# Prayforhanluo/HiCHap_master

Measured on NVIDIA B200. Metric: matrix_stage_time_to_ice_convergence, lower is better.
Workload: dtype int32 counts (ICE streams them as u8 + overflow list, s32 tensor-core plane sums) / f64 weights

## Files before the change

### hichap_master_b200/csrc/hc_ice.cu

```cuda
#include <cooperative_groups.h>
#include <vector>
#include <algorithm>
#include <math.h>
#include <stdlib.h>
#include "hc_common.cuh"
#include "hc_select.cuh"

namespace {

__device__ __forceinline__ double band_weight(int j, int r, int kd) {
    const int d = j - r;
    if (d == 0) return kd == 0 ? 2.0 : 0.0;
    return (d < kd && d > -kd) ? 0.0 : 1.0;
}

__global__ void __launch_bounds__(256)
ice_dense_marginals_kernel(const int32_t* __restrict__ mats, const int64_t* __restrict__ mat_off,
                           const int32_t* __restrict__ mat_n, const int32_t* __restrict__ mat_ld,
                           const int64_t* __restrict__ bin_off, int nprob, int kd,
                           double* __restrict__ nnz_marg, double* __restrict__ marg) {
    const int64_t g = ((int64_t)blockIdx.x * blockDim.x + threadIdx.x) >> 5;
    const int lane = threadIdx.x & 31;
    if (g >= bin_off[nprob]) return;
    int p = 0;
// ... 216 lines not shown
    }
    if (!mad_last_cta(st, &flag_s)) return;
    if (threadIdx.x == 0) {
        const long long k = mad_median_rank(count);
        const long long le_all = *reinterpret_cast<volatile long long*>(&st->le);
        const unsigned long long nxt_all = *reinterpret_cast<volatile unsigned long long*>(&st->nxt);
        const double lo = key_f64(klo);
        double hi = lo;
        if (k + 1 < count && le_all < k + 2) hi = key_f64(nxt_all);
        st->result[STAGE] = (count & 1) ? lo : __dmul_rn(__dadd_rn(lo, hi), 0.5);
    }
}

__global__ void __launch_bounds__(MAD_THREADS)
mad_apply_kernel(const double* __restrict__ marg, long long n, double mad_max, const MadState* __restrict__ st,
                 double* __restrict__ bias) {
    const double cutoff = exp(__dadd_rn(st->result[0], -__dmul_rn(mad_max, st->result[1])));
    for (long long i = (long long)blockIdx.x * blockDim.x + threadIdx.x; i < n; i += (long long)gridDim.x * blockDim.x)
        if (marg[i] < cutoff) bias[i] = 0.0;
}

struct IceDenseArgs {
    const int32_t* mats; const int64_t* mat_off; const int32_t* mat_n; const int32_t* mat_ld;
    const int64_t* pad_off;
    const int32_t* item_prob; const int32_t* item_row0; const int32_t* item_nrows;
    const unsigned int* nitems; unsigned int* queue;
    int32_t* iter;
    double* bias;
    double* marg;
    hc_ice_result* results; int32_t* done; int32_t* n_done;
    double tol; int kd; int max_iters; int nprob;
    unsigned int queue_start;
    const uint8_t* q8; const int64_t* q_off;
    uint8_t* digits; int32_t* dig_exp;
    const int4* desc; int kseg;
    double* part; int nseg_max; long long npad;
    const int64_t* bin_off;
    const int64_t* ovf_ptr; const int32_t* ovf_col; const int32_t* ovf_val;
    int packed;
};

template <int RG>
__device__ __forceinline__ void consume_chunk(const int4 (&a)[RG], const double* __restrict__ b, int j, int jc,
                                              int rg, int kd, int kspan, double (&acc)[RG]) {
    const double2 b01 = *reinterpret_cast<const double2*>(b + j);
    const double2 b23 = *reinterpret_cast<const double2*>(b + j + 2);
    const bool band = jc <= rg + RG - 1 + kspan && jc + 127 >= rg - kspan;
#pragma unroll
    for (int q = 0; q < RG; ++q) {
        double x0 = (double)a[q].x, x1 = (double)a[q].y, x2 = (double)a[q].z, x3 = (double)a[q].w;
        if (band) {
            const int r = rg + q;
            x0 *= band_weight(j, r, kd); x1 *= band_weight(j + 1, r, kd);
            x2 *= band_weight(j + 2, r, kd); x3 *= band_weight(j + 3, r, kd);
        }
        acc[q] = fma(x0, b01.x, acc[q]); acc[q] = fma(x1, b01.y, acc[q]);
        acc[q] = fma(x2, b23.x, acc[q]); acc[q] = fma(x3, b23.y, acc[q]);
    }
}

template <int RG, int U, int MINB>
__global__ void __launch_bounds__(256, MINB)
ice_dense_stream_kernel(IceDenseArgs A) {
    const int lane = threadIdx.x & 31;
    const int kd = A.kd, kspan = kd > 0 ? kd - 1 : 0;
    const unsigned nitems = *A.nitems;
// ... 33 lines not shown
                        for (int q = 0; q < RG; ++q) a[u][q] = ld_stream_v4(base + roff[q] + (c0 + u) * 128);
#pragma unroll
                    for (int u = 0; u < U; ++u)
                        consume_chunk<RG>(a[u], b, (c0 + u) * 128 + 4 * lane, (c0 + u) * 128, rg, kd, kspan, acc);
                }
                for (; c0 < nchunk; ++c0) {
                    int4 a[RG];
#pragma unroll
                    for (int q = 0; q < RG; ++q) a[q] = ld_stream_v4(base + roff[q] + c0 * 128);
                    consume_chunk<RG>(a, b, c0 * 128 + 4 * lane, c0 * 128, rg, kd, kspan, acc);
                }
#pragma unroll
                for (int q = 0; q < RG; ++q) {
                    const double sacc = warp_sum(acc[q]);
                    if (lane == 0 && q < nr) mout[rg + q] = b[rg + q] * sacc;
                }
            }
        }
        item = __shfl_sync(0xffffffffu, next, 0);
    }
}

__device__ __forceinline__ long long weighted_count(int v, int j, int r, int kd) {
    const int d = j - r;
    if (d == 0) return kd == 0 ? 2ll * v : 0ll;
    return (d < kd && d > -kd) ? 0ll : (long long)v;
}

__global__ void __launch_bounds__(256)
ice_pack_tiles_kernel(const int32_t* __restrict__ mats, const int64_t* __restrict__ mat_off,
                      const int32_t* __restrict__ mat_n, const int32_t* __restrict__ mat_ld,
                      const int64_t* __restrict__ q_off, const int64_t* __restrict__ strip_off,
                      const int64_t* __restrict__ bin_off, int nprob, int kd, uint8_t* __restrict__ q8,
                      unsigned long long* __restrict__ ovf_cnt, int32_t* __restrict__ ovf_lo, int32_t* __restrict__ ovf_hi) {
    const int64_t gs = ((int64_t)blockIdx.x * blockDim.x + threadIdx.x) >> 5;
    const int lane = threadIdx.x & 31;
    if (gs >= strip_off[nprob]) return;
    int p = 0;
    while (p + 1 < nprob && strip_off[p + 1] <= gs) ++p;
    const int sidx = (int)(gs - strip_off[p]), n = mat_n[p], ld = mat_ld[p], KT = ld >> 5;
    const int32_t* M = mats + mat_off[p];
    uint8_t* out = q8 + q_off[p] + (int64_t)sidx * KT * 512 + 16 * lane;
    const int g = lane >> 2, c = 4 * (lane & 3);
    const int ra = sidx * 16 + g, rb = ra + 8;
    const int64_t grow = bin_off[p] + sidx * 16;
    for (int t = 8 * blockIdx.y; t < min(KT, 8 * (int)blockIdx.y + 8); ++t) {
        uint32_t w[4];
#pragma unroll
        for (int h = 0; h < 4; ++h) {
            const int r = (h & 1) ? rb : ra, j0 = t * 32 + ((h & 2) ? 16 : 0) + c;
            uint32_t word = 0;
            if (r < n) {
                const int4 a = ld_stream_v4(M + (int64_t)r * ld + j0);
                const int x[4] = {a.x, a.y, a.z, a.w};
#pragma unroll
                for (int e = 0; e < 4; ++e) {
                    const long long wc = (j0 + e < n) ? weighted_count(x[e], j0 + e, r, kd) : 0ll;
                    if (wc > 255) {
                        const int64_t gr = grow + (r - sidx * 16);
                        atomicAdd(ovf_cnt + gr, 1ull);
                        atomicMin(ovf_lo + gr, j0 + e);
                        atomicMax(ovf_hi + gr, j0 + e);
                    }
                    word |= (uint32_t)(wc > 255 ? 255 : (wc < 0 ? 0 : wc)) << (8 * e);
                }
            }
            w[h] = word;
        }
        *reinterpret_cast<uint4*>(out + (int64_t)t * 512) = make_uint4(w[0], w[1], w[2], w[3]);
    }
}

__device__ __forceinline__ void ice_store_digits(const double (&bv)[4], int j4, double pow2, uint32_t* __restrict__ dw) {
    unsigned long long F[4];
#pragma unroll
    for (int e = 0; e < 4; ++e) F[e] = bv[e] > 0.0 ? __double2ull_rn(bv[e] * pow2) : 0ull;
    const int t = j4 >> 5, cc = j4 & 31, sub = (cc & 15) >> 2, reg = cc >> 4;
#pragma unroll
    for (int pl = 0; pl < 8; ++pl) {
        const int sh = 8 * (7 - pl);
        const uint32_t word = (uint32_t)((F[0] >> sh) & 255ull) | ((uint32_t)((F[1] >> sh) & 255ull) << 8) |
                              ((uint32_t)((F[2] >> sh) & 255ull) << 16) | ((uint32_t)((F[3] >> sh) & 255ull) << 24);
        dw[t * 64 + (pl * 4 + sub) * 2 + reg] = word;
    }
}

__device__ __forceinline__ double block_max(double v, double* red) {
#pragma unroll
    for (int o = 16; o > 0; o >>= 1) v = fmax(v, __shfl_xor_sync(0xffffffffu, v, o));
    __syncthreads();
    if ((threadIdx.x & 31) == 0) red[threadIdx.x >> 5] = v;
    __syncthreads();
    double t = 0.0;
    for (int w = 0; w < (int)(blockDim.x >> 5); ++w) t = fmax(t, red[w]);
    return t;
}

__device__ __forceinline__ int digits_exponent(double mx, double* pow2) {
    const int E = (mx > 1.0e-300 && mx < 1.0e300) ? (int)((__double_as_longlong(mx) >> 52) & 0x7ff) - 1023 + 1 : 0;
    *pow2 = __longlong_as_double((long long)(1023 + 64 - E) << 52);
    return E;
}
// ... 79 lines not shown
                    int32_t* __restrict__ ovf_col, int32_t* __restrict__ ovf_val) {
    const int64_t g = ((int64_t)blockIdx.x * blockDim.x + threadIdx.x) >> 5;
    const int lane = threadIdx.x & 31;
    if (g >= bin_off[nprob]) return;
    int64_t out = ovf_ptr[g];
    if (ovf_ptr[g + 1] == out) return;
    int p = 0;
    while (p + 1 < nprob && bin_off[p + 1] <= g) ++p;
    const int r = (int)(g - bin_off[p]);
    const int32_t* row = mats + mat_off[p] + (int64_t)r * mat_ld[p];
    const int hi = ovf_hi[g];
    for (int j0 = ovf_lo[g]; j0 <= hi; j0 += 32) {
        const int j = j0 + lane;
        const long long w = j <= hi ? weighted_count(row[j], j, r, kd) : 0ll;
        const unsigned m = __ballot_sync(0xffffffffu, w > 255);
        if (w > 255) {
            const int64_t at = out + __popc(m & ((1u << lane) - 1u));
            ovf_col[at] = j;
            ovf_val[at] = (int32_t)(w - 255);
        }
        out += __popc(m);
    }
}

__device__ __forceinline__ void mma_u8(int (&c)[4], const int4& a, const uint2& b) {
    asm volatile("mma.sync.aligned.m16n8k32.row.col.s32.u8.u8.s32 {%0,%1,%2,%3}, {%4,%5,%6,%7}, {%8,%9}, {%0,%1,%2,%3};"
                 : "+r"(c[0]), "+r"(c[1]), "+r"(c[2]), "+r"(c[3])
                 : "r"(a.x), "r"(a.y), "r"(a.z), "r"(a.w), "r"(b.x), "r"(b.y));
}

template <int RS, int U, int MINB>
__global__ void __launch_bounds__(256, MINB)
ice_q8_mma_kernel(IceDenseArgs A) {
    const int lane = threadIdx.x & 31;
    const int g = lane >> 2, t4 = lane & 3;
    const double w_even = __longlong_as_double((long long)(1023 + 8 * (7 - 2 * t4)) << 52);
    const double w_odd = __longlong_as_double((long long)(1023 + 8 * (6 - 2 * t4)) << 52);
    const unsigned nitems = *A.nitems;
    unsigned cur = (blockIdx.x * 256u + threadIdx.x) >> 5;
    unsigned nxt = 0;
    if (lane == 0) {
        nxt = atomicAdd(A.queue, 1u);
        if (cur == 0) atomicAdd(A.iter, 1);
    }
    int4 d0 = make_int4(0, 0, 0, 0), d1 = d0, d2 = d0, d3 = d0;
    if (cur < nitems) {
        const int4* dp = A.desc + 4 * (int64_t)A.item_prob[cur];
        d0 = __ldg(dp); d1 = __ldg(dp + 1); d2 = __ldg(dp + 2); d3 = __ldg(dp + 3);
    }
    nxt = __shfl_sync(0xffffffffu, nxt, 0);
    while (cur < nitems) {
        unsigned drawn = 0;
        if (lane == 0) drawn = atomicAdd(A.queue, 1u);
        int4 e0 = make_int4(0, 0, 0, 0), e1 = e0, e2 = e0, e3 = e0;
        if (nxt < nitems) {
            const int4* dp = A.desc + 4 * (int64_t)A.item_prob[nxt];
            e0 = __ldg(dp); e1 = __ldg(dp + 1); e2 = __ldg(dp + 2); e3 = __ldg(dp + 3);
        }
        const int p = d2.x;
        if (!A.done[p]) {
            const int64_t tile_off = ((int64_t)(uint32_t)d0.x) | ((int64_t)d0.y << 32);
            const int64_t part_base = ((int64_t)(uint32_t)d0.z) | ((int64_t)d0.w << 32);
            const int64_t dig_off = ((int64_t)(uint32_t)d1.x) | ((int64_t)d1.y << 32);
            const int64_t grow = ((int64_t)(uint32_t)d1.z) | ((int64_t)d1.w << 32);
            const int nrows = d2.w, nk = d3.x, seg = d3.y, KT = d3.z;
            const uint8_t* qp = A.q8 + tile_off + 16 * lane;
            const uint8_t* dig = A.digits + dig_off + 8 * lane;
            const double* __restrict__ b = A.bias + d2.y;
            const double scale = __longlong_as_double((long long)(1023 + A.dig_exp[p] - 64) << 52);
            double* pout = A.part + part_base;
            const int ns = min(RS, (nrows + 15) >> 4);
            const uint8_t* sp[RS];
#pragma unroll
            for (int s = 0; s < RS; ++s) sp[s] = qp + (int64_t)min(s, ns - 1) * KT * 512;
            int c[RS][4];
#pragma unroll
            for (int s = 0; s < RS; ++s) { c[s][0] = 0; c[s][1] = 0; c[s][2] = 0; c[s][3] = 0; }
            for (int t = 0; t < nk; t += U) {
                int4 a[U][RS];
                uint2 bf[U];
#pragma unroll
                for (int u = 0; u < U; ++u) {
                    const int tt = min(t + u, nk - 1);
#pragma unroll
                    for (int s = 0; s < RS; ++s)
                        a[u][s] = ld_stream_v4(reinterpret_cast<const int32_t*>(sp[s] + (int64_t)tt * 512));
                    bf[u] = t + u < nk ? *reinterpret_cast<const uint2*>(dig + (int64_t)tt * 256) : make_uint2(0u, 0u);
                }
#pragma unroll
                for (int u = 0; u < U; ++u)
#pragma unroll
                    for (int s = 0; s < RS; ++s) mma_u8(c[s], a[u][s], bf[u]);
            }
#pragma unroll
            for (int s = 0; s < RS; ++s) {
                if (s < ns) {
                    const int ra = 16 * s + g, rb = ra + 8;
                    double va = ((double)c[s][0] * w_even + (double)c[s][1] * w_odd) * scale;
                    double vb = ((double)c[s][2] * w_even + (double)c[s][3] * w_odd) * scale;
                    if (seg == 0) {
                        if (ra < nrows) {
                            const int64_t x0 = A.ovf_ptr[grow + ra], x1 = A.ovf_ptr[grow + ra + 1];
                            for (int64_t e = x0 + t4; e < x1; e += 4) va = fma((double)A.ovf_val[e], b[A.ovf_col[e]], va);
                        }
                        if (rb < nrows) {
                            const int64_t x0 = A.ovf_ptr[grow + rb], x1 = A.ovf_ptr[grow + rb + 1];
                            for (int64_t e = x0 + t4; e < x1; e += 4) vb = fma((double)A.ovf_val[e], b[A.ovf_col[e]], vb);
                        }
                    }
                    va += __shfl_xor_sync(0xffffffffu, va, 1); va += __shfl_xor_sync(0xffffffffu, va, 2);
                    vb += __shfl_xor_sync(0xffffffffu, vb, 1); vb += __shfl_xor_sync(0xffffffffu, vb, 2);
                    if (t4 == 0) {
                        if (ra < nrows) pout[ra] = va;
                        if (rb < nrows) pout[rb] = vb;
                    }
                }
            }
        }
        cur = nxt; d0 = e0; d1 = e1; d2 = e2; d3 = e3;
        nxt = __shfl_sync(0xffffffffu, drawn, 0);
    }
}

__global__ void __launch_bounds__(1024)
ice_dense_update_kernel(IceDenseArgs A) {
    __shared__ double red[32];
    __shared__ long long redll[32];
    const int p = blockIdx.x;
    const int k = *A.iter;
    if (p == 0 && threadIdx.x == 0) *A.queue = A.queue_start;
    if (A.done[p] || k > A.max_iters) return;
    const int n = A.mat_n[p];
    if (n == 0) return;
    const int64_t lo = A.pad_off[p];
    double* m_in = A.marg + lo;
    double* bw = A.bias + lo;
    const double nan = __longlong_as_double(0x7ff8000000000000ll);
    if (A.packed && n <= 8 * (int)blockDim.x) {
        const int nseg = ((A.mat_ld[p] >> 5) + A.kseg - 1) / A.kseg;
        const int ld = A.mat_ld[p];
        const double* part = A.part + lo;
        double m[8], bb[8];
        double s = 0.0;
        long long c = 0;
        const int ja = 4 * threadIdx.x, jb = 4 * (int)blockDim.x + 4 * threadIdx.x;
        const bool ina = ja < ld, inb = jb < ld;
#pragma unroll
        for (int i = 0; i < 8; ++i) m[i] = 0.0;
#pragma unroll
// ... 239 lines not shown
    int p = 0;
    while (p + 1 < nprob && bin_off[p + 1] <= g) ++p;
    padded[pad_off[p] + (g - bin_off[p])] = bias[g];
}

__global__ void __launch_bounds__(256)
ice_finalize_kernel(const int64_t* __restrict__ bin_off, const int64_t* __restrict__ pad_off, int nprob,
                    const hc_ice_result* __restrict__ results, int rescale, const double* __restrict__ padded,
                    double* __restrict__ bias) {
    const int64_t g = (int64_t)blockIdx.x * blockDim.x + threadIdx.x;
    if (g >= bin_off[nprob]) return;
    int p = 0;
    while (p + 1 < nprob && bin_off[p + 1] <= g) ++p;
    const hc_ice_result r = results[p];
    const double nan = __longlong_as_double(0x7ff8000000000000ll);
    double b = padded[pad_off[p] + (g - bin_off[p])];
    if (isnan(r.scale)) b = nan;
    else {
        if (b == 0.0) b = nan;
        if (rescale) b = b / sqrt(r.scale);
    }
    bias[g] = b;
}

struct Scratch {
    cudaStream_t s;
    std::vector<void*> ptrs;
    explicit Scratch(cudaStream_t st) : s(st) {}
    cudaError_t alloc(void** p, size_t bytes) {
        const cudaError_t e = cudaMallocAsync(p, bytes, s);
        if (e == cudaSuccess) ptrs.push_back(*p);
        return e;
    }
    ~Scratch() { for (void* p : ptrs) cudaFreeAsync(p, s); }
};
struct EventPair {
    cudaEvent_t a = nullptr, b = nullptr;
    void create() { cudaEventCreate(&a); cudaEventCreate(&b); }
    ~EventPair() { if (a) cudaEventDestroy(a); if (b) cudaEventDestroy(b); }
};

typedef void (*StreamKernel)(IceDenseArgs);
struct StreamVariant { StreamKernel fn; int rg, u, minb; };
const StreamVariant kVariants[] = {
    {ice_dense_stream_kernel<4, 2, 4>, 4, 2, 4},
    {ice_dense_stream_kernel<4, 2, 3>, 4, 2, 3},
    {ice_dense_stream_kernel<2, 2, 4>, 2, 2, 4},
    {ice_dense_stream_kernel<2, 4, 3>, 2, 4, 3},
    {ice_dense_stream_kernel<4, 4, 2>, 4, 4, 2},
    {ice_dense_stream_kernel<1, 4, 4>, 1, 4, 4},
};

const StreamVariant kQ8Variants[] = {
    {ice_q8_mma_kernel<2, 4, 4>, 32, 4, 4},
    {ice_q8_mma_kernel<1, 4, 4>, 16, 4, 4},
    {ice_q8_mma_kernel<1, 8, 3>, 16, 8, 3},
    {ice_q8_mma_kernel<2, 4, 3>, 32, 4, 3},
    {ice_q8_mma_kernel<1, 8, 4>, 16, 8, 4},
    {ice_q8_mma_kernel<2, 8, 2>, 32, 8, 2},
    {ice_q8_mma_kernel<1, 16, 2>, 16, 16, 2},
    {ice_q8_mma_kernel<1, 12, 3>, 16, 12, 3},
};

}

extern "C" int hc_ice_dense_marginals(const int32_t* mats, const int64_t* mat_off, const int32_t* mat_n,
                                      const int32_t* mat_ld, const int64_t* bin_off, int32_t nprob,
                                      int32_t ignore_diags, double* nnz_marg, double* marg, void* stream) {
    HC_REQUIRE(nprob > 0 && ignore_diags >= 0, "nprob>0, ignore_diags>=0");
    int64_t total = 0;
    HC_CUDA(hc_read_small(&total, bin_off + nprob, sizeof(int64_t), (cudaStream_t)stream));
    if (total == 0) return HC_OK;
    const int64_t blocks = (total * 32 + 255) / 256;
    ice_dense_marginals_kernel<<<(unsigned)blocks, 256, 0, (cudaStream_t)stream>>>(
        mats, mat_off, mat_n, mat_ld, bin_off, nprob, ignore_diags, nnz_marg, marg);
    HC_LAUNCH_CHECK();
    return HC_OK;
}

extern "C" int hc_ice_filter_bins(const double* nnz_marg, double* marg, int64_t nbins, const int64_t* chrom_off,
                                  int32_t nchrom, const hc_ice_params* P, double* bias, double* work, void* stream) {
    HC_REQUIRE(nbins >= 0 && nchrom > 0 && P != nullptr, "nbins>=0, nchrom>0, params");
    if (nbins == 0) return HC_OK;
    const int do_mad = P->mad_max > 0.0;
    ice_filter_chrom_kernel<<<nchrom, 1024, 0, (cudaStream_t)stream>>>(nnz_marg, marg, chrom_off, P->min_nnz,
                                                                      P->min_count, do_mad, bias);
    HC_LAUNCH_CHECK();
    if (do_mad) {
        const char* e_single = getenv("HC_ICE_MAD_SINGLE");
        const bool single = e_single ? atoi(e_single) != 0 : nbins < 8192;
        if (single) {
            ice_filter_mad_kernel<<<1, 1024, 0, (cudaStream_t)stream>>>(marg, nbins, P->mad_max, bias, work);
            HC_LAUNCH_CHECK();
            return HC_OK;
// ... 35 lines not shown
                                    const int32_t* h_mat_n, const hc_ice_params* P, double* bias,
                                    hc_ice_result* results, hc_ice_run_info* h_info, void* stream) {
    HC_REQUIRE(nprob > 0 && h_mat_n != nullptr && P != nullptr, "nprob>0, h_mat_n, params");
    HC_REQUIRE(P->max_iters >= 1 && P->ignore_diags >= 0, "max_iters>=1, ignore_diags>=0");
    int64_t nbins = 0;
    for (int p = 0; p < nprob; ++p) {
        HC_REQUIRE(h_mat_n[p] >= 0, "matrix side");
        nbins += h_mat_n[p];
    }
    if (h_info) { h_info->launches = 0; h_info->loop_ms = 0.f; h_info->packed = 0; h_info->pack_ms = 0.f; h_info->overflow_cells = 0; h_info->stream_full_ms = 0.f; h_info->stream_full_launches = 0; }
    if (nbins == 0) return HC_OK;
    static thread_local cudaStream_t private_stream[64] = {nullptr};
    int dev = 0;
    HC_CUDA(cudaGetDevice(&dev));
    HC_REQUIRE(dev >= 0 && dev < 64, "device index");
    if (!private_stream[dev]) HC_CUDA(cudaStreamCreateWithFlags(&private_stream[dev], cudaStreamNonBlocking));
    cudaStream_t s = private_stream[dev];
    {
        cudaEvent_t e_in;
        HC_CUDA(cudaEventCreateWithFlags(&e_in, cudaEventDisableTiming));
        HC_CUDA(cudaEventRecord(e_in, (cudaStream_t)stream));
        HC_CUDA(cudaStreamWaitEvent(s, e_in, 0));
        cudaEventDestroy(e_in);
    }

    bool packed = true;
    if (const char* e = getenv("HC_ICE_PACKED")) packed = atoi(e) != 0;
    int64_t total_rows = 0;
    for (int p = 0; p < nprob; ++p) total_rows += h_mat_n[p];
    StreamVariant V;
    if (packed) {
        int vi = -1;
        if (const char* e = getenv("HC_ICE_Q8_VARIANT")) vi = atoi(e);
        if (vi < 0 || vi >= (int)(sizeof(kQ8Variants) / sizeof(kQ8Variants[0]))) vi = 6;
        V = kQ8Variants[vi];
    } else {
        int vi = -1;
        if (const char* e = getenv("HC_ICE_VARIANT")) vi = atoi(e);
        if (vi < 0 || vi >= (int)(sizeof(kVariants) / sizeof(kVariants[0]))) {
            const int64_t warps = (int64_t)hc_num_sms() * 4 * 8;
            vi = total_rows / 4 >= warps + warps / 4 ? 0 : (total_rows / 2 >= warps + warps / 4 ? 2 : 5);
        }
        V = kVariants[vi];
    }
    int item_kb = 32;
    if (const char* e = getenv("HC_ICE_ITEM_KB")) item_kb = std::max(1, atoi(e));
    int kseg = 48;
    if (const char* e = getenv("HC_ICE_KSEG")) kseg = std::min(1024, std::max(4, atoi(e) / 4 * 4));
    else if (packed) {
        const int64_t warps = (int64_t)hc_num_sms() * V.minb * 8;
        for (;;) {
            int64_t items = 0;
            for (int p = 0; p < nprob; ++p) items += (int64_t)((h_mat_n[p] + V.rg - 1) / V.rg) * (((h_mat_n[p] + 127) / 128 * 4 + kseg - 1) / kseg);
            if (items >= 4 * warps || kseg <= 16) break;
            kseg -= 16;
        }
    }

    std::vector<int32_t> h_ld(nprob);
    HC_CUDA(hc_read_small(h_ld.data(), mat_ld, sizeof(int32_t) * nprob, s));
    std::vector<int64_t> h_pad(nprob + 1, 0);
    for (int p = 0; p < nprob; ++p) {
        if (h_ld[p] < h_mat_n[p] || (h_ld[p] & 127) != 0) {
            hc_set_error("hc_ice_dense_balance: ld must be >= n and a multiple of 128 elements (matrix %d: n=%d ld=%d)",
                         p, h_mat_n[p], h_ld[p]);
            return HC_ERR_ARG;
        }
        h_pad[p + 1] = h_pad[p] + h_ld[p];
    }
    const int64_t npad = h_pad[nprob];

    std::vector<int32_t> h_done(nprob, 0);
    std::vector<int32_t> item_prob, item_row0, item_nrows;
    std::vector<int4> item_desc;
    bool desc_built = false;
    std::vector<int> desc_lo(nprob, 0), desc_hi(nprob, 0);
    std::vector<int64_t> h_qoff(nprob, 0), h_binoff(nprob + 1, 0);
    if (packed) {
        int64_t qb = 0;
        for (int p = 0; p < nprob; ++p) {
            h_qoff[p] = qb;
            qb += (int64_t)((h_mat_n[p] + 15) / 16) * 16 * h_ld[p];
            h_binoff[p + 1] = h_binoff[p] + h_mat_n[p];
        }
    }
    int nseg_max = 1;
    for (int p = 0; p < nprob; ++p) nseg_max = std::max(nseg_max, ((h_ld[p] >> 5) + kseg - 1) / kseg);
    auto build_items = [&]() {
        item_prob.clear(); item_row0.clear(); item_nrows.clear();
        std::vector<int> order(nprob);
        for (int p = 0; p < nprob; ++p) order[p] = p;
        std::stable_sort(order.begin(), order.end(), [&](int a, int b) { return h_mat_n[a] > h_mat_n[b]; });
        for (int p : order) {
            const int n = h_mat_n[p];
            if (n == 0 || h_done[p]) continue;
            if (packed) {
                const int KT = h_ld[p] >> 5;
                auto lohi = [](int64_t v, int& a, int& b) { a = (int)(uint32_t)(v & 0xffffffffll); b = (int)(v >> 32); };
                if (desc_built) {
                    for (int id = desc_lo[p]; id < desc_hi[p]; ++id) { item_prob.push_back(id); item_row0.push_back(0); item_nrows.push_back(0); }
                    continue;
                }
                for (int r0 = 0; r0 < n; r0 += V.rg)
                    for (int k0 = 0; k0 < KT; k0 += kseg) {
                        item_prob.push_back((int)(item_desc.size() / 4)); item_row0.push_back(r0); item_nrows.push_back(std::min(V.rg, n - r0));
                        int4 d0, d1, d2, d3;
                        lohi(h_qoff[p] + ((int64_t)(r0 / 16) * KT + k0) * 512, d0.x, d0.y);
                        lohi((int64_t)(k0 / kseg) * npad + h_pad[p] + r0, d0.z, d0.w);
                        lohi(8 * h_pad[p] + (int64_t)k0 * 256, d1.x, d1.y);
                        lohi(h_binoff[p] + r0, d1.z, d1.w);
                        d2 = make_int4(p, (int)h_pad[p], r0, std::min(V.rg, n - r0));
                        d3 = make_int4(std::min(kseg, KT - k0), k0 / kseg, KT, 0);
                        item_desc.push_back(d0); item_desc.push_back(d1); item_desc.push_back(d2); item_desc.push_back(d3);
                    }
                continue;
            }
            int rows = (int)((int64_t)item_kb * 1024 / ((int64_t)h_ld[p] * 4));
            rows = std::max(V.rg, rows / V.rg * V.rg);
            for (int r0 = 0; r0 < n; r0 += rows) {
                item_prob.push_back(p); item_row0.push_back(r0); item_nrows.push_back(std::min(rows, n - r0));
            }
        }
    };
    build_items();
    const size_t max_items = item_prob.size();
    if (packed) {
        desc_built = true;
        std::vector<int> cnt(nprob, 0);
        for (size_t i = 0; i < item_desc.size(); i += 4) cnt[item_desc[i + 2].x]++;
        std::vector<int> order(nprob);
        for (int p = 0; p < nprob; ++p) order[p] = p;
        std::stable_sort(order.begin(), order.end(), [&](int a, int b) { return h_mat_n[a] > h_mat_n[b]; });
        int run = 0;
        for (int p : order) { desc_lo[p] = run; run += cnt[p]; desc_hi[p] = run; }
    }

    Scratch scratch(s);
    double* d_vec = nullptr;
    HC_CUDA(scratch.alloc((void**)&d_vec, (2 * (size_t)npad + nprob + 1) * sizeof(double)));
    double* biasp = d_vec;
    double* marg = d_vec + npad;
    int64_t* d_pad = reinterpret_cast<int64_t*>(d_vec + 2 * npad);
    HC_CUDA(cudaMemsetAsync(d_vec, 0, 2 * (size_t)npad * sizeof(double), s));
    HC_CUDA(cudaMemcpyAsync(d_pad, h_pad.data(), (nprob + 1) * sizeof(int64_t), cudaMemcpyHostToDevice, s));
    ice_pad_bias_kernel<<<(unsigned)((nbins + 255) / 256), 256, 0, s>>>(bin_off, d_pad, nprob, bias, biasp);
    HC_LAUNCH_CHECK();

    uint8_t* d_q8 = nullptr;
    int64_t* d_ovf_ptr = nullptr;
    int32_t* d_ovf = nullptr;
    uint8_t* d_digits = nullptr;
    double* d_part = nullptr;
    int64_t* d_qoff = nullptr;
    int32_t* d_exp = nullptr;
    long long novf = 0;
    EventPair evp;
    cudaEvent_t& evp0 = evp.a;
    cudaEvent_t& evp1 = evp.b;
    if (packed) {
        if (h_info) { evp.create(); cudaEventRecord(evp0, s); }
        std::vector<int64_t> h_q(2 * (size_t)nprob + 1);
        int64_t qbytes = 0, strips = 0;
        for (int p = 0; p < nprob; ++p) {
            h_q[p] = qbytes;
            h_q[nprob + p] = strips;
            const int64_t sp = (h_mat_n[p] + 15) / 16;
            qbytes += sp * 16 * h_ld[p];
            strips += sp;
        }
        h_q[2 * (size_t)nprob] = strips;
        HC_CUDA(scratch.alloc((void**)&d_q8, (size_t)qbytes + 8 * (size_t)npad * (1 + (size_t)nseg_max) + 16));
        d_digits = d_q8 + ((qbytes + 15) & ~15ll);
        d_part = reinterpret_cast<double*>(d_digits + 8 * (size_t)npad);
        const size_t ptr_bytes = ((size_t)nbins + 1 + 2 * (size_t)nprob + 1 + (size_t)((nbins + 1023) / 1024) + 1) * sizeof(int64_t);
        HC_CUDA(scratch.alloc((void**)&d_ovf_ptr, ptr_bytes + (2 * (size_t)nbins + nprob) * sizeof(int32_t)));
        d_qoff = d_ovf_ptr + nbins + 1;
        int64_t* d_strip = d_qoff + nprob;
        int32_t* d_lo = reinterpret_cast<int32_t*>(reinterpret_cast<unsigned char*>(d_ovf_ptr) + ptr_bytes);
        int32_t* d_hi = d_lo + nbins;
        d_exp = d_hi + nbins;
        HC_CUDA(cudaMemcpyAsync(d_qoff, h_q.data(), h_q.size() * sizeof(int64_t), cudaMemcpyHostToDevice, s));
        HC_CUDA(cudaMemsetAsync(d_ovf_ptr, 0, ((size_t)nbins + 1) * sizeof(int64_t), s));
        HC_CUDA(cudaMemsetAsync(d_lo, 0x7f, (size_t)nbins * sizeof(int32_t), s));
        HC_CUDA(cudaMemsetAsync(d_hi, 0xff, (size_t)nbins * sizeof(int32_t), s));
        HC_CUDA(cudaStreamSynchronize(s));
        int kt_max = 0;
        for (int p = 0; p < nprob; ++p) kt_max = std::max(kt_max, h_ld[p] >> 5);
        ice_pack_tiles_kernel<<<dim3((unsigned)((strips * 32 + 255) / 256), (unsigned)((kt_max + 7) / 8)), 256, 0, s>>>(
            mats, mat_off, mat_n, mat_ld, d_qoff, d_strip, bin_off, nprob, P->ignore_diags, d_q8,
            reinterpret_cast<unsigned long long*>(d_ovf_ptr), d_lo, d_hi);
        HC_LAUNCH_CHECK();
        {
            const int nb = (int)((nbins + 1023) / 1024);
            int64_t* d_bsum = d_strip + nprob + 1;
            ice_ovf_blocksum_kernel<<<nb, 256, 0, s>>>(d_ovf_ptr, nbins, d_bsum);
            HC_LAUNCH_CHECK();
            ice_ovf_scan_blocks_kernel<<<1, 1024, 0, s>>>(d_bsum, nb);
            HC_LAUNCH_CHECK();
            ice_ovf_scan_kernel<<<nb, 256, 0, s>>>(d_ovf_ptr, nbins, d_bsum, nb);
            HC_LAUNCH_CHECK();
        }
        HC_CUDA(hc_read_small(&novf, d_ovf_ptr + nbins, sizeof(long long), s));
        HC_CUDA(scratch.alloc((void**)&d_ovf, 2 * (size_t)std::max(novf, 1ll) * sizeof(int32_t)));
        if (novf > 0) {
            ice_pack_ovf_kernel<<<(unsigned)((nbins * 32 + 255) / 256), 256, 0, s>>>(
                mats, mat_off, mat_n, mat_ld, bin_off, nprob, P->ignore_diags, d_ovf_ptr, d_lo, d_hi, d_ovf, d_ovf + novf);
            HC_LAUNCH_CHECK();
        }
    }
    int32_t* d_tab = nullptr;
    const size_t desc_at = (3 * max_items + (size_t)nprob + 4 + 3) & ~(size_t)3;
    const size_t tab_ints = desc_at + (packed ? 16 * max_items : 0);
    HC_CUDA(scratch.alloc((void**)&d_tab, tab_ints * sizeof(int32_t)));
    bool desc_uploaded = false;
    auto upload_items = [&]() -> cudaError_t {
        const size_t n = item_prob.size();
        const int32_t n32 = (int32_t)n;
        cudaError_t e = cudaMemcpyAsync(d_tab + 3 * max_items + nprob + 3, &n32, sizeof(int32_t), cudaMemcpyHostToDevice, s);
        if (e == cudaSuccess) e = cudaMemcpyAsync(d_tab, item_prob.data(), n * sizeof(int32_t), cudaMemcpyHostToDevice, s);
        if (e == cudaSuccess) e = cudaMemcpyAsync(d_tab + max_items, item_row0.data(), n * sizeof(int32_t), cudaMemcpyHostToDevice, s);
        if (e == cudaSuccess) e = cudaMemcpyAsync(d_tab + 2 * max_items, item_nrows.data(), n * sizeof(int32_t), cudaMemcpyHostToDevice, s);
        if (e == cudaSuccess && packed && !desc_uploaded) {
            e = cudaMemcpyAsync(d_tab + desc_at, item_desc.data(), item_desc.size() * sizeof(int4), cudaMemcpyHostToDevice, s);
            desc_uploaded = true;
        }
        if (e == cudaSuccess) e = cudaStreamSynchronize(s);
        return e;
    };
    HC_CUDA(cudaMemsetAsync(d_tab + 3 * max_items, 0, ((size_t)nprob + 3) * sizeof(int32_t), s));
    HC_CUDA(upload_items());
    const int grid = hc_num_sms() * V.minb;
    const unsigned int queue_start = (unsigned)grid * 8u;
    HC_CUDA(cudaMemcpyAsync(d_tab + 3 * max_items + nprob + 1, &queue_start, sizeof(unsigned int), cudaMemcpyHostToDevice, s));

    IceDenseArgs A;
    A.mats = mats; A.mat_off = mat_off; A.mat_n = mat_n; A.mat_ld = mat_ld; A.pad_off = d_pad;
    A.item_prob = d_tab; A.item_row0 = d_tab + max_items; A.item_nrows = d_tab + 2 * max_items;
    A.done = d_tab + 3 * max_items;
    A.n_done = A.done + nprob;
    A.queue = reinterpret_cast<unsigned int*>(A.n_done + 1);
    A.iter = A.n_done + 2;
    A.nitems = reinterpret_cast<const unsigned int*>(A.n_done + 3);
    A.bias = biasp; A.marg = marg; A.results = results;
    A.tol = P->tol; A.kd = P->ignore_diags; A.max_iters = P->max_iters; A.nprob = nprob; A.queue_start = queue_start;
    A.q8 = d_q8; A.q_off = d_qoff; A.digits = d_digits; A.dig_exp = d_exp; A.packed = packed ? 1 : 0;
    A.desc = reinterpret_cast<const int4*>(d_tab + desc_at); A.kseg = kseg; A.part = d_part; A.nseg_max = nseg_max; A.npad = npad;
    A.bin_off = bin_off; A.ovf_ptr = d_ovf_ptr; A.ovf_col = d_ovf; A.ovf_val = d_ovf ? d_ovf + novf : nullptr;
    if (packed) {
        ice_digits_kernel<<<nprob, 1024, 0, s>>>(A);
        HC_LAUNCH_CHECK();
        if (evp0) cudaEventRecord(evp1, s);
    }

    int nonempty = 0;
    for (int p = 0; p < nprob; ++p) nonempty += h_mat_n[p] > 0;
    if (nonempty != nprob) {
        std::vector<hc_ice_result> h_res(nprob);
        for (int p = 0; p < nprob; ++p) { h_res[p].scale = NAN; h_res[p].var = 0.0; h_res[p].iters = 0; h_res[p].converged = 1; }
        HC_CUDA(cudaMemcpyAsync(results, h_res.data(), sizeof(hc_ice_result) * nprob, cudaMemcpyHostToDevice, s));
        HC_CUDA(cudaStreamSynchronize(s));
    }
    const size_t smem = 0;
    cudaFuncSetAttribute(V.fn, cudaFuncAttributePreferredSharedMemoryCarveout, cudaSharedmemCarveoutMaxL1);
    bool cluster_update = packed;
    for (int p = 0; p < nprob; ++p) cluster_update = cluster_update && h_ld[p] <= UPD_CLUSTER * 256 * 4;
    if (const char* e = getenv("HC_ICE_CLUSTER_UPDATE")) cluster_update = cluster_update && atoi(e) != 0;
    auto launch_update = [&]() {
        if (cluster_update) ice_q8_update_cluster_kernel<<<nprob * UPD_CLUSTER, 256, 0, s>>>(A);
        else ice_dense_update_kernel<<<nprob, 1024, 0, s>>>(A);
    };
    const int poll = P->poll_every > 0 ? P->poll_every : 8;
    int launches = 0, h_ndone = 0, seen_done = 0;
    int rc = HC_OK;
    cudaGraphExec_t gexec = nullptr;
    bool use_graph = true;
    if (const char* e = getenv("HC_ICE_GRAPH")) use_graph = atoi(e) != 0;
    struct GraphCache {
        cudaGraphExec_t exec = nullptr;
// ... 116 lines not shown
```

Measured before the change: 12.53.

## Compress ICE u8 tiles into skipped-zero, nibble and byte super-tile classes

New measurement: 12.12, median of 6. -3.2%, faster.

```diff
diff --git a/hichap_master_b200/csrc/hc_ice.cu b/hichap_master_b200/csrc/hc_ice.cu
--- a/hichap_master_b200/csrc/hc_ice.cu
+++ b/hichap_master_b200/csrc/hc_ice.cu
@@ -272,6 +272,7 @@
     double tol; int kd; int max_iters; int nprob;
     unsigned int queue_start;
     const uint8_t* q8; const int64_t* q_off;
+    const int64_t* tile_base; const int2* tile_cnt; const uint16_t* tidx;
     uint8_t* digits; int32_t* dig_exp;
     const int4* desc; int kseg;
     double* part; int nseg_max; long long npad;
@@ -371,7 +372,8 @@
                       const int32_t* __restrict__ mat_n, const int32_t* __restrict__ mat_ld,
                       const int64_t* __restrict__ q_off, const int64_t* __restrict__ strip_off,
                       const int64_t* __restrict__ bin_off, int nprob, int kd, uint8_t* __restrict__ q8,
-                      unsigned long long* __restrict__ ovf_cnt, int32_t* __restrict__ ovf_lo, int32_t* __restrict__ ovf_hi) {
+                      uint8_t* __restrict__ cls, unsigned long long* __restrict__ ovf_cnt, int32_t* __restrict__ ovf_lo,
+                      int32_t* __restrict__ ovf_hi) {
     const int64_t gs = ((int64_t)blockIdx.x * blockDim.x + threadIdx.x) >> 5;
     const int lane = threadIdx.x & 31;
     if (gs >= strip_off[nprob]) return;
@@ -383,6 +385,8 @@
     const int g = lane >> 2, c = 4 * (lane & 3);
     const int ra = sidx * 16 + g, rb = ra + 8;
     const int64_t grow = bin_off[p] + sidx * 16;
+    uint8_t* cl = cls + q_off[p] / 1024 + (int64_t)sidx * (KT >> 1);
+    unsigned mx = 0;
     for (int t = 8 * blockIdx.y; t < min(KT, 8 * (int)blockIdx.y + 8); ++t) {
         uint32_t w[4];
 #pragma unroll
@@ -401,12 +405,84 @@
                         atomicMin(ovf_lo + gr, j0 + e);
                         atomicMax(ovf_hi + gr, j0 + e);
                     }
-                    word |= (uint32_t)(wc > 255 ? 255 : (wc < 0 ? 0 : wc)) << (8 * e);
+                    const uint32_t q = (uint32_t)(wc > 255 ? 255 : (wc < 0 ? 0 : wc));
+                    mx = q > mx ? q : mx;
+                    word |= q << (8 * e);
                 }
             }
             w[h] = word;
         }
         *reinterpret_cast<uint4*>(out + (int64_t)t * 512) = make_uint4(w[0], w[1], w[2], w[3]);
+        if (t & 1) {
+            mx = __reduce_max_sync(0xffffffffu, mx);
+            if (lane == 0) cl[t >> 1] = mx == 0 ? 0 : (mx <= 15 ? 1 : 2);
+            mx = 0;
+        }
+    }
+}
+
+__global__ void __launch_bounds__(256)
+ice_tile_lists_kernel(const int32_t* __restrict__ mat_ld, const int64_t* __restrict__ q_off,
+                      const int64_t* __restrict__ strip_off, int nprob, const uint8_t* __restrict__ cls,
+                      uint16_t* __restrict__ tidx, int32_t* __restrict__ rel, int2* __restrict__ cnt,
+                      int64_t* __restrict__ sbytes) {
+    const int64_t gs = ((int64_t)blockIdx.x * blockDim.x + threadIdx.x) >> 5;
+    const int lane = threadIdx.x & 31;
+    if (gs >= strip_off[nprob]) return;
+    int p = 0;
+    while (p + 1 < nprob && strip_off[p + 1] <= gs) ++p;
+    const int ST = mat_ld[p] >> 6;
+    const int64_t g0 = q_off[p] / 1024 + (gs - strip_off[p]) * ST;
+    int n8 = 0, n4 = 0;
+    for (int j0 = 0; j0 < ST; j0 += 32) {
+        const int c = j0 + lane < ST ? cls[g0 + j0 + lane] : 0;
+        n8 += __popc(__ballot_sync(0xffffffffu, c == 2));
+        n4 += __popc(__ballot_sync(0xffffffffu, c == 1));
+    }
+    int i8 = 0, i4 = n8;
+    const unsigned below = (1u << lane) - 1u;
+    for (int j0 = 0; j0 < ST; j0 += 32) {
+        const int j = j0 + lane;
+        const int c = j < ST ? cls[g0 + j] : 0;
+        const unsigned m8 = __ballot_sync(0xffffffffu, c == 2), m4 = __ballot_sync(0xffffffffu, c == 1);
+        if (j < ST) {
+            int at = -1;
+            if (c == 2) at = i8 + __popc(m8 & below);
+            if (c == 1) at = i4 + __popc(m4 & below);
+            if (at >= 0) tidx[g0 + at] = (uint16_t)j;
+            rel[g0 + j] = c == 2 ? at * 1024 : (c == 1 ? n8 * 1024 + (at - n8) * 512 : -1);
+        }
+        i8 += __popc(m8); i4 += __popc(m4);
+    }
+    if (lane == 0) { cnt[gs] = make_int2(n8, n4); sbytes[gs] = (int64_t)n8 * 1024 + (int64_t)n4 * 512; }
+}
+
+__global__ void __launch_bounds__(256)
+ice_compact_tiles_kernel(const int32_t* __restrict__ mat_ld, const int64_t* __restrict__ q_off,
+                         const int64_t* __restrict__ strip_off, int nprob, const uint8_t* __restrict__ q8tmp,
+                         const uint8_t* __restrict__ cls, const int32_t* __restrict__ rel, const int64_t* __restrict__ sbase,
+                         uint8_t* __restrict__ q8) {
+    const int64_t gs = ((int64_t)blockIdx.x * blockDim.x + threadIdx.x) >> 5;
+    const int lane = threadIdx.x & 31;
+    if (gs >= strip_off[nprob]) return;
+    int p = 0;
+    while (p + 1 < nprob && strip_off[p + 1] <= gs) ++p;
+    const int ST = mat_ld[p] >> 6;
+    const int64_t g0 = q_off[p] / 1024 + (gs - strip_off[p]) * ST;
+    const uint8_t* src = q8tmp + g0 * 1024 + 16 * lane;
+    uint8_t* dst = q8 + sbase[gs] + 16 * lane;
+    for (int i = 8 * blockIdx.y; i < min(ST, 8 * (int)blockIdx.y + 8); ++i) {
+        const int c = cls[g0 + i];
+        if (c == 0) continue;
+        const int r = rel[g0 + i];
+        const int4 a = ld_stream_v4(reinterpret_cast<const int32_t*>(src + (int64_t)i * 1024));
+        const int4 b = ld_stream_v4(reinterpret_cast<const int32_t*>(src + (int64_t)i * 1024 + 512));
+        if (c == 2) {
+            *reinterpret_cast<int4*>(dst + r) = a;
+            *reinterpret_cast<int4*>(dst + r + 512) = b;
+        } else {
+            *reinterpret_cast<int4*>(dst + r) = make_int4(a.x | (b.x << 4), a.y | (b.y << 4), a.z | (b.z << 4), a.w | (b.w << 4));
+        }
     }
 }
 
@@ -552,6 +628,8 @@
 template <int RS, int U, int MINB>
 __global__ void __launch_bounds__(256, MINB)
 ice_q8_mma_kernel(IceDenseArgs A) {
+    static_assert(RS == 1, "one strip per work item: every strip has its own tile runs");
+    static_assert(U % 2 == 0 && U <= 32, "U: even, at most one tile list entry per lane");
     const int lane = threadIdx.x & 31;
     const int g = lane >> 2, t4 = lane & 3;
     const double w_even = __longlong_as_double((long long)(1023 + 8 * (7 - 2 * t4)) << 52);
@@ -579,62 +657,85 @@
         }
         const int p = d2.x;
         if (!A.done[p]) {
-            const int64_t tile_off = ((int64_t)(uint32_t)d0.x) | ((int64_t)d0.y << 32);
+            const int strip = d0.x;
             const int64_t part_base = ((int64_t)(uint32_t)d0.z) | ((int64_t)d0.w << 32);
             const int64_t dig_off = ((int64_t)(uint32_t)d1.x) | ((int64_t)d1.y << 32);
             const int64_t grow = ((int64_t)(uint32_t)d1.z) | ((int64_t)d1.w << 32);
-            const int nrows = d2.w, nk = d3.x, seg = d3.y, KT = d3.z;
-            const uint8_t* qp = A.q8 + tile_off + 16 * lane;
+            const int nrows = d2.w, nseg = d3.x, seg = d3.y;
+            const int2 cnt = __ldg(A.tile_cnt + strip);
+            const int n8 = cnt.x, n4 = cnt.y;
+            const uint8_t* q8 = A.q8 + __ldg(A.tile_base + strip) + 16 * lane;
+            const uint8_t* q4 = q8 + (int64_t)n8 * 1024;
+            const uint16_t* ix = A.tidx + (uint32_t)d0.y;
             const uint8_t* dig = A.digits + dig_off + 8 * lane;
             const double* __restrict__ b = A.bias + d2.y;
             const double scale = __longlong_as_double((long long)(1023 + A.dig_exp[p] - 64) << 52);
             double* pout = A.part + part_base;
-            const int ns = min(RS, (nrows + 15) >> 4);
-            const uint8_t* sp[RS];
-#pragma unroll
-            for (int s = 0; s < RS; ++s) sp[s] = qp + (int64_t)min(s, ns - 1) * KT * 512;
-            int c[RS][4];
-#pragma unroll
-            for (int s = 0; s < RS; ++s) { c[s][0] = 0; c[s][1] = 0; c[s][2] = 0; c[s][3] = 0; }
-            for (int t = 0; t < nk; t += U) {
-                int4 a[U][RS];
-                uint2 bf[U];
+            const int cost = 2 * n8 + n4;
+            const int lo = (int)((int64_t)seg * cost / nseg), hi = (int)((int64_t)(seg + 1) * cost / nseg);
+            const int i8a = min(n8, (lo + 1) >> 1), i8b = min(n8, (hi + 1) >> 1);
+            const int i4a = max(0, lo - 2 * n8), i4b = max(0, hi - 2 * n8);
+            int c[4] = {0, 0, 0, 0};
+            constexpr int U8 = U / 2;
+            for (int i = i8a; i < i8b; i += U8) {
+                const int my = (lane < U8 && i + lane < i8b) ? (int)__ldg(ix + i + lane) : 0;
+                int4 a[U8][2];
+#pragma unroll
+                for (int u = 0; u < U8; ++u) {
+                    const int tt = min(i + u, i8b - 1);
+                    a[u][0] = ld_stream_v4(reinterpret_cast<const int32_t*>(q8 + (int64_t)tt * 1024));
+                    a[u][1] = ld_stream_v4(reinterpret_cast<const int32_t*>(q8 + (int64_t)tt * 1024 + 512));
+                }
+#pragma unroll
+                for (int u = 0; u < U8; ++u) {
+                    const int st = __shfl_sync(0xffffffffu, my, u);
+                    uint2 b0 = make_uint2(0u, 0u), b1 = b0;
+                    if (i + u < i8b) {
+                        b0 = *reinterpret_cast<const uint2*>(dig + (int64_t)st * 512);
+                        b1 = *reinterpret_cast<const uint2*>(dig + (int64_t)st * 512 + 256);
+                    }
+                    mma_u8(c, a[u][0], b0);
+                    mma_u8(c, a[u][1], b1);
+                }
+            }
+            for (int j = i4a; j < i4b; j += U) {
+                const int my = (lane < U && j + lane < i4b) ? (int)__ldg(ix + n8 + j + lane) : 0;
+                int4 a[U];
+#pragma unroll
+                for (int u = 0; u < U; ++u)
+                    a[u] = ld_stream_v4(reinterpret_cast<const int32_t*>(q4 + (int64_t)min(j + u, i4b - 1) * 512));
 #pragma unroll
                 for (int u = 0; u < U; ++u) {
-                    const int tt = min(t + u, nk - 1);
-#pragma unroll
-                    for (int s = 0; s < RS; ++s)
-                        a[u][s] = ld_stream_v4(reinterpret_cast<const int32_t*>(sp[s] + (int64_t)tt * 512));
-                    bf[u] = t + u < nk ? *reinterpret_cast<const uint2*>(dig + (int64_t)tt * 256) : make_uint2(0u, 0u);
+                    const int st = __shfl_sync(0xffffffffu, my, u);
+                    uint2 b0 = make_uint2(0u, 0u), b1 = b0;
+                    if (j + u < i4b) {
+                        b0 = *reinterpret_cast<const uint2*>(dig + (int64_t)st * 512);
+                        b1 = *reinterpret_cast<const uint2*>(dig + (int64_t)st * 512 + 256);
+                    }
+                    const int4 w = a[u];
+                    mma_u8(c, make_int4(w.x & 0x0F0F0F0F, w.y & 0x0F0F0F0F, w.z & 0x0F0F0F0F, w.w & 0x0F0F0F0F), b0);
+                    mma_u8(c, make_int4((w.x >> 4) & 0x0F0F0F0F, (w.y >> 4) & 0x0F0F0F0F, (w.z >> 4) & 0x0F0F0F0F,
+                                        (w.w >> 4) & 0x0F0F0F0F), b1);
                 }
-#pragma unroll
-                for (int u = 0; u < U; ++u)
-#pragma unroll
-                    for (int s = 0; s < RS; ++s) mma_u8(c[s], a[u][s], bf[u]);
-            }
-#pragma unroll
-            for (int s = 0; s < RS; ++s) {
-                if (s < ns) {
-                    const int ra = 16 * s + g, rb = ra + 8;
-                    double va = ((double)c[s][0] * w_even + (double)c[s][1] * w_odd) * scale;
-                    double vb = ((double)c[s][2] * w_even + (double)c[s][3] * w_odd) * scale;
-                    if (seg == 0) {
-                        if (ra < nrows) {
-                            const int64_t x0 = A.ovf_ptr[grow + ra], x1 = A.ovf_ptr[grow + ra + 1];
-                            for (int64_t e = x0 + t4; e < x1; e += 4) va = fma((double)A.ovf_val[e], b[A.ovf_col[e]], va);
-                        }
-                        if (rb < nrows) {
-                            const int64_t x0 = A.ovf_ptr[grow + rb], x1 = A.ovf_ptr[grow + rb + 1];
-                            for (int64_t e = x0 + t4; e < x1; e += 4) vb = fma((double)A.ovf_val[e], b[A.ovf_col[e]], vb);
-                        }
-                    }
-                    va += __shfl_xor_sync(0xffffffffu, va, 1); va += __shfl_xor_sync(0xffffffffu, va, 2);
-                    vb += __shfl_xor_sync(0xffffffffu, vb, 1); vb += __shfl_xor_sync(0xffffffffu, vb, 2);
-                    if (t4 == 0) {
-                        if (ra < nrows) pout[ra] = va;
-                        if (rb < nrows) pout[rb] = vb;
-                    }
+            }
+            const int ra = g, rb = g + 8;
+            double va = ((double)c[0] * w_even + (double)c[1] * w_odd) * scale;
+            double vb = ((double)c[2] * w_even + (double)c[3] * w_odd) * scale;
+            if (seg == 0) {
+                if (ra < nrows) {
+                    const int64_t x0 = A.ovf_ptr[grow + ra], x1 = A.ovf_ptr[grow + ra + 1];
+                    for (int64_t e = x0 + t4; e < x1; e += 4) va = fma((double)A.ovf_val[e], b[A.ovf_col[e]], va);
                 }
+                if (rb < nrows) {
+                    const int64_t x0 = A.ovf_ptr[grow + rb], x1 = A.ovf_ptr[grow + rb + 1];
+                    for (int64_t e = x0 + t4; e < x1; e += 4) vb = fma((double)A.ovf_val[e], b[A.ovf_col[e]], vb);
+                }
+            }
+            va += __shfl_xor_sync(0xffffffffu, va, 1); va += __shfl_xor_sync(0xffffffffu, va, 2);
+            vb += __shfl_xor_sync(0xffffffffu, vb, 1); vb += __shfl_xor_sync(0xffffffffu, vb, 2);
+            if (t4 == 0) {
+                if (ra < nrows) pout[ra] = va;
+                if (rb < nrows) pout[rb] = vb;
             }
         }
         cur = nxt; d0 = e0; d1 = e1; d2 = e2; d3 = e3;
@@ -940,6 +1041,10 @@
         if (e == cudaSuccess) ptrs.push_back(*p);
         return e;
     }
+    cudaError_t release(void* p) {
+        ptrs.erase(std::find(ptrs.begin(), ptrs.end(), p));
+        return cudaFreeAsync(p, s);
+    }
     ~Scratch() { for (void* p : ptrs) cudaFreeAsync(p, s); }
 };
 struct EventPair {
@@ -960,14 +1065,9 @@
 };
 
 const StreamVariant kQ8Variants[] = {
-    {ice_q8_mma_kernel<2, 4, 4>, 32, 4, 4},
-    {ice_q8_mma_kernel<1, 4, 4>, 16, 4, 4},
-    {ice_q8_mma_kernel<1, 8, 3>, 16, 8, 3},
-    {ice_q8_mma_kernel<2, 4, 3>, 32, 4, 3},
-    {ice_q8_mma_kernel<1, 8, 4>, 16, 8, 4},
-    {ice_q8_mma_kernel<2, 8, 2>, 32, 8, 2},
     {ice_q8_mma_kernel<1, 16, 2>, 16, 16, 2},
-    {ice_q8_mma_kernel<1, 12, 3>, 16, 12, 3},
+    {ice_q8_mma_kernel<1, 8, 2>, 16, 8, 2},
+    {ice_q8_mma_kernel<1, 12, 2>, 16, 12, 2},
 };
 
 }
@@ -1069,7 +1169,7 @@
     if (packed) {
         int vi = -1;
         if (const char* e = getenv("HC_ICE_Q8_VARIANT")) vi = atoi(e);
-        if (vi < 0 || vi >= (int)(sizeof(kQ8Variants) / sizeof(kQ8Variants[0]))) vi = 6;
+        if (vi < 0 || vi >= (int)(sizeof(kQ8Variants) / sizeof(kQ8Variants[0]))) vi = 0;
         V = kQ8Variants[vi];
     } else {
         int vi = -1;
@@ -1112,14 +1212,17 @@
     std::vector<int4> item_desc;
     bool desc_built = false;
     std::vector<int> desc_lo(nprob, 0), desc_hi(nprob, 0);
-    std::vector<int64_t> h_qoff(nprob, 0), h_binoff(nprob + 1, 0);
+    std::vector<int64_t> h_qoff(nprob, 0), h_binoff(nprob + 1, 0), h_soff(nprob + 1, 0);
     if (packed) {
         int64_t qb = 0;
         for (int p = 0; p < nprob; ++p) {
+            HC_REQUIRE(h_ld[p] / 64 <= 65536, "packed ICE: at most 65536 super-tiles of 64 columns per row");
             h_qoff[p] = qb;
             qb += (int64_t)((h_mat_n[p] + 15) / 16) * 16 * h_ld[p];
             h_binoff[p + 1] = h_binoff[p] + h_mat_n[p];
-        }
+            h_soff[p + 1] = h_soff[p] + (h_mat_n[p] + 15) / 16;
+        }
+        HC_REQUIRE(qb / 1024 < INT32_MAX, "packed ICE: super-tile index range");
     }
     int nseg_max = 1;
     for (int p = 0; p < nprob; ++p) nseg_max = std::max(nseg_max, ((h_ld[p] >> 5) + kseg - 1) / kseg);
@@ -1138,16 +1241,18 @@
                     for (int id = desc_lo[p]; id < desc_hi[p]; ++id) { item_prob.push_back(id); item_row0.push_back(0); item_nrows.push_back(0); }
                     continue;
                 }
+                const int nseg = (KT + kseg - 1) / kseg;
                 for (int r0 = 0; r0 < n; r0 += V.rg)
-                    for (int k0 = 0; k0 < KT; k0 += kseg) {
+                    for (int q = 0; q < nseg; ++q) {
                         item_prob.push_back((int)(item_desc.size() / 4)); item_row0.push_back(r0); item_nrows.push_back(std::min(V.rg, n - r0));
                         int4 d0, d1, d2, d3;
-                        lohi(h_qoff[p] + ((int64_t)(r0 / 16) * KT + k0) * 512, d0.x, d0.y);
-                        lohi((int64_t)(k0 / kseg) * npad + h_pad[p] + r0, d0.z, d0.w);
-                        lohi(8 * h_pad[p] + (int64_t)k0 * 256, d1.x, d1.y);
+                        d0.x = (int)(h_soff[p] + r0 / 16);
+                        d0.y = (int)((h_qoff[p] + (int64_t)(r0 / 16) * 16 * h_ld[p]) / 1024);
+                        lohi((int64_t)q * npad + h_pad[p] + r0, d0.z, d0.w);
+                        lohi(8 * h_pad[p], d1.x, d1.y);
                         lohi(h_binoff[p] + r0, d1.z, d1.w);
                         d2 = make_int4(p, (int)h_pad[p], r0, std::min(V.rg, n - r0));
-                        d3 = make_int4(std::min(kseg, KT - k0), k0 / kseg, KT, 0);
+                        d3 = make_int4(nseg, q, 0, 0);
                         item_desc.push_back(d0); item_desc.push_back(d1); item_desc.push_back(d2); item_desc.push_back(d3);
                     }
                 continue;
@@ -1186,6 +1291,9 @@
     uint8_t* d_q8 = nullptr;
     int64_t* d_ovf_ptr = nullptr;
     int32_t* d_ovf = nullptr;
+    int64_t* d_tbase = nullptr;
+    int2* d_tcnt = nullptr;
+    uint16_t* d_tidx = nullptr;
     uint8_t* d_digits = nullptr;
     double* d_part = nullptr;
     int64_t* d_qoff = nullptr;
@@ -1206,9 +1314,17 @@
             strips += sp;
         }
         h_q[2 * (size_t)nprob] = strips;
-        HC_CUDA(scratch.alloc((void**)&d_q8, (size_t)qbytes + 8 * (size_t)npad * (1 + (size_t)nseg_max) + 16));
-        d_digits = d_q8 + ((qbytes + 15) & ~15ll);
-        d_part = reinterpret_cast<double*>(d_digits + 8 * (size_t)npad);
+        const int64_t nst = qbytes / 1024;
+        const int nbs = (int)((strips + 1023) / 1024);
+        uint8_t* d_tmp = nullptr;
+        HC_CUDA(scratch.alloc((void**)&d_tmp, (size_t)qbytes));
+        const size_t i64s = (size_t)strips + 1 + (size_t)nbs + 1;
+        HC_CUDA(scratch.alloc((void**)&d_tbase, i64s * sizeof(int64_t) + (size_t)strips * sizeof(int2) + (size_t)nst * (4 + 2 + 1)));
+        int64_t* d_tbsum = d_tbase + strips + 1;
+        d_tcnt = reinterpret_cast<int2*>(d_tbase + i64s);
+        int32_t* d_rel = reinterpret_cast<int32_t*>(d_tcnt + strips);
+        d_tidx = reinterpret_cast<uint16_t*>(d_rel + nst);
+        uint8_t* d_cls = reinterpret_cast<uint8_t*>(d_tidx + nst);
         const size_t ptr_bytes = ((size_t)nbins + 1 + 2 * (size_t)nprob + 1 + (size_t)((nbins + 1023) / 1024) + 1) * sizeof(int64_t);
         HC_CUDA(scratch.alloc((void**)&d_ovf_ptr, ptr_bytes + (2 * (size_t)nbins + nprob) * sizeof(int32_t)));
         d_qoff = d_ovf_ptr + nbins + 1;
@@ -1223,9 +1339,12 @@
         HC_CUDA(cudaStreamSynchronize(s));
         int kt_max = 0;
         for (int p = 0; p < nprob; ++p) kt_max = std::max(kt_max, h_ld[p] >> 5);
-        ice_pack_tiles_kernel<<<dim3((unsigned)((strips * 32 + 255) / 256), (unsigned)((kt_max + 7) / 8)), 256, 0, s>>>(
-            mats, mat_off, mat_n, mat_ld, d_qoff, d_strip, bin_off, nprob, P->ignore_diags, d_q8,
+        const unsigned sblocks = (unsigned)((strips * 32 + 255) / 256);
+        ice_pack_tiles_kernel<<<dim3(sblocks, (unsigned)((kt_max + 7) / 8)), 256, 0, s>>>(
+            mats, mat_off, mat_n, mat_ld, d_qoff, d_strip, bin_off, nprob, P->ignore_diags, d_tmp, d_cls,
             reinterpret_cast<unsigned long long*>(d_ovf_ptr), d_lo, d_hi);
+        HC_LAUNCH_CHECK();
+        ice_tile_lists_kernel<<<sblocks, 256, 0, s>>>(mat_ld, d_qoff, d_strip, nprob, d_cls, d_tidx, d_rel, d_tcnt, d_tbase);
         HC_LAUNCH_CHECK();
         {
             const int nb = (int)((nbins + 1023) / 1024);
@@ -1236,8 +1355,23 @@
             HC_LAUNCH_CHECK();
             ice_ovf_scan_kernel<<<nb, 256, 0, s>>>(d_ovf_ptr, nbins, d_bsum, nb);
             HC_LAUNCH_CHECK();
-        }
+            ice_ovf_blocksum_kernel<<<nbs, 256, 0, s>>>(d_tbase, strips, d_tbsum);
+            HC_LAUNCH_CHECK();
+            ice_ovf_scan_blocks_kernel<<<1, 1024, 0, s>>>(d_tbsum, nbs);
+            HC_LAUNCH_CHECK();
+            ice_ovf_scan_kernel<<<nbs, 256, 0, s>>>(d_tbase, strips, d_tbsum, nbs);
+            HC_LAUNCH_CHECK();
+        }
+        long long tbytes = 0;
         HC_CUDA(hc_read_small(&novf, d_ovf_ptr + nbins, sizeof(long long), s));
+        HC_CUDA(hc_read_small(&tbytes, d_tbase + strips, sizeof(long long), s));
+        HC_CUDA(scratch.alloc((void**)&d_q8, (size_t)tbytes + 8 * (size_t)npad * (1 + (size_t)nseg_max) + 16));
+        d_digits = d_q8 + ((tbytes + 15) & ~15ll);
+        d_part = reinterpret_cast<double*>(d_digits + 8 * (size_t)npad);
+        ice_compact_tiles_kernel<<<dim3(sblocks, (unsigned)((kt_max / 2 + 7) / 8)), 256, 0, s>>>(
+            mat_ld, d_qoff, d_strip, nprob, d_tmp, d_cls, d_rel, d_tbase, d_q8);
+        HC_LAUNCH_CHECK();
+        HC_CUDA(scratch.release(d_tmp));
         HC_CUDA(scratch.alloc((void**)&d_ovf, 2 * (size_t)std::max(novf, 1ll) * sizeof(int32_t)));
         if (novf > 0) {
             ice_pack_ovf_kernel<<<(unsigned)((nbins * 32 + 255) / 256), 256, 0, s>>>(
@@ -1280,7 +1414,7 @@
     A.nitems = reinterpret_cast<const unsigned int*>(A.n_done + 3);
     A.bias = biasp; A.marg = marg; A.results = results;
     A.tol = P->tol; A.kd = P->ignore_diags; A.max_iters = P->max_iters; A.nprob = nprob; A.queue_start = queue_start;
-    A.q8 = d_q8; A.q_off = d_qoff; A.digits = d_digits; A.dig_exp = d_exp; A.packed = packed ? 1 : 0;
+    A.q8 = d_q8; A.q_off = d_qoff; A.tile_base = d_tbase; A.tile_cnt = d_tcnt; A.tidx = d_tidx; A.digits = d_digits; A.dig_exp = d_exp; A.packed = packed ? 1 : 0;
     A.desc = reinterpret_cast<const int4*>(d_tab + desc_at); A.kseg = kseg; A.part = d_part; A.nseg_max = nseg_max; A.npad = npad;
     A.bin_off = bin_off; A.ovf_ptr = d_ovf_ptr; A.ovf_col = d_ovf; A.ovf_val = d_ovf ? d_ovf + novf : nullptr;
     if (packed) {
diff --git a/profiles/ice_tile_classes.py b/profiles/ice_tile_classes.py
--- /dev/null
+++ b/profiles/ice_tile_classes.py
@@ -0,0 +1,118 @@
+import argparse
+import json
+import os
+import subprocess
+import sys
+
+ROOT = os.path.dirname(os.path.dirname(os.path.abspath(__file__)))
+sys.path.insert(0, ROOT)
+
+
+def card():
+    try:
+        q = subprocess.run(["nvidia-smi", "-i", "0", "--query-gpu=name,power.limit", "--format=csv,noheader"],
+                           capture_output=True, text=True, timeout=30).stdout.strip()
+        name, power = [x.strip() for x in q.split(",")]
+        return name, power
+    except Exception:
+        return None, None
+
+
+def tile_classes(view, n, ld, kd):
+    import torch
+    rows = (n + 15) // 16 * 16
+    w = torch.zeros((rows, ld), dtype=torch.int64, device=view.device)
+    w[:n] = view.to(torch.int64)
+    i = torch.arange(rows, device=view.device)[:, None]
+    j = torch.arange(ld, device=view.device)[None, :]
+    d = (j - i).abs()
+    w = torch.where(d < kd, torch.zeros_like(w), w)
+    if kd == 0:
+        w = torch.where(d == 0, 2 * w, w)
+    mx = w.view(rows // 16, 16, ld // 64, 64).amax(dim=(1, 3))
+    return int((mx == 0).sum()), int(((mx > 0) & (mx <= 15)).sum()), int((mx > 15).sum())
+
+
+def main():
+    ap = argparse.ArgumentParser()
+    ap.add_argument("--pairs", type=int, default=400_000_000)
+    ap.add_argument("--steps", type=int, default=10)
+    ap.add_argument("--warmup", type=int, default=3)
+    ap.add_argument("--out", default=None)
+    args = ap.parse_args()
+
+    import torch
+    import bench
+    from hichap_master_b200 import kernels, synth
+    from hichap_master_b200.device import PairColumns
+    from hichap_master_b200.pipeline import LocalStage
+
+    assert torch.cuda.is_available(), "needs a GPU"
+    dev = torch.device("cuda", 0)
+    torch.cuda.set_device(0)
+    genome, order = bench.c2_genome()
+    sizes = [genome[c] // bench.RES + 1 for c in order]
+    shares = bench.pair_shares(genome, order, args.pairs)
+    cs, p1s, p2s = [], [], []
+    for li, c in enumerate(order):
+        _, a, _, b = synth.genome_pairs_torch({c: genome[c]}, [c], int(shares[li]), 2000 + li, dev)
+        cs.append(torch.full((a.numel(),), li, dtype=torch.int32, device=dev)); p1s.append(a); p2s.append(b)
+    c1 = torch.cat(cs); p1 = torch.cat(p1s); p2 = torch.cat(p2s)
+    del cs, p1s, p2s
+    g = torch.Generator(device=dev); g.manual_seed(99)
+    perm = torch.randperm(c1.numel(), generator=g, device=dev)
+    c1, p1, p2 = c1[perm].contiguous(), p1[perm].contiguous(), p2[perm].contiguous()
+    del perm
+    pairs = PairColumns(c1, p1, c1, p2, device=dev)
+    stage = LocalStage(sizes, int(c1.numel()), dev)
+
+    os.environ.setdefault("HC_ICE_TIME_KERNEL", "1")
+    step = lambda: stage.run(pairs, bench.RES, records=False, weights_to_host=False)
+    for _ in range(args.warmup):
+        step()
+    torch.cuda.synchronize()
+    e0, e1 = torch.cuda.Event(enable_timing=True), torch.cuda.Event(enable_timing=True)
+    e0.record()
+    for _ in range(args.steps):
+        out = step()
+    e1.record()
+    torch.cuda.synchronize()
+    step_ms = e0.elapsed_time(e1) / args.steps
+    info = out["info"]
+
+    kd = int(kernels.ice_params().ignore_diags)
+    batch = stage.batch
+    z = q4 = q8 = 0
+    for i in range(len(sizes)):
+        a, b, c = tile_classes(batch.view(i), batch.sizes[i], batch.lds[i], kd)
+        z += a; q4 += b; q8 += c
+    tiles = z + q4 + q8
+    cells = float(sum(n * n for n in sizes))
+    ovf = int(info.overflow_cells)
+    enc_bytes = 1024.0 * q8 + 512.0 * q4 + 2.0 * (q8 + q4) + 8.0 * ovf
+    u8_bytes = 1.0 * cells + 8.0 * ovf
+    peaks = bench.load_peaks()
+    peak = float(peaks.get("hbm_gbs", 0.0)) or None
+    kms = float(info.stream_full_ms)
+    gbs = enc_bytes / (kms * 1e6) if kms > 0 else None
+    name, power = card()
+    res = {
+        "card": name, "power_limit": power, "pairs": args.pairs, "steps": args.steps,
+        "step_ms": step_ms, "loop_ms": float(info.loop_ms), "stream_full_ms": kms,
+        "stream_full_launches": int(info.stream_full_launches), "pack_ms": float(info.pack_ms),
+        "ignore_diags": kd, "super_tiles": tiles,
+        "share_zero": z / tiles, "share_nibble": q4 / tiles, "share_u8": q8 / tiles,
+        "overflow_cells": ovf, "bytes_per_launch": enc_bytes, "bytes_per_cell": enc_bytes / cells,
+        "u8_encoding_bytes_per_launch": u8_bytes,
+        "achieved_GBps": gbs, "peak_GBps": peak, "peak_source": "MEASURED_PEAKS.json hbm_gbs" if peak else None,
+        "frac_of_peak": (gbs / peak) if (gbs and peak) else None,
+    }
+    line = json.dumps(res)
+    print(line)
+    if args.out:
+        with open(args.out, "w") as f:
+            f.write(line + "\n")
+
+
+if __name__ == "__main__":
+    main()
```
